# penn-graphics-research/claymore

Measured on AMD Instinct MI355X. Metric: particles*steps/sec, higher is better.
Workload: dtype f32

## Files before the change

claymore_amd/csrc/claymore_hip.hip:

```cpp
#include <hip/hip_runtime.h>

#include <algorithm>
#include <cmath>
#include <cstdio>
#include <cstdlib>
#include <chrono>
#include <cstring>
#include <string>
#include <vector>

#include "../../include/claymore_amd.h"
#include "mpm_kernels.hpp"
#include "mpm_readout.hpp"

using namespace mpm;

namespace {
constexpr int kHaloWords	 = 128;
constexpr int kStatusBlock = ST_WORDS + kHaloWords + kMaxVelSlots * kMaxVelStride;

struct Partition {
	int* table = nullptr;
	int* keys  = nullptr;
	int* count = nullptr;
// ... 26 lines not shown

}

struct SubstepEvents {
	hipEvent_t start = nullptr, g2p2g_start = nullptr, g2p2g_end = nullptr, end = nullptr;
};

struct mpm_ctx {
	mpm_config cfg {};
	GridCfg g {};
	int device = 0;
	hipStream_t s_compute = nullptr, s_comm = nullptr;
	SubstepEvents ev;
	hipEvent_t ev_comm = nullptr, ev_halo = nullptr;
	hipEvent_t ev_tag0 = nullptr, ev_tag1 = nullptr;
	bool lean_events = false;
	hipEvent_t ev_pending = nullptr;
	hipEvent_t ev_status = nullptr;
	bool grid_preupdated = false;
	bool grid_momentum = false;
	float preupdate_dt	 = 0.f;
	float fuse_dt_once	 = 0.f;
	bool rebuild_cleared = false;
	std::vector<hipEvent_t> ev_ring;
	Partition part[2];
	float* grid[2] = {nullptr, nullptr};
	int rollid	   = 0;
	int pbc = 0, nbc = 0, ebc = 0;
	int pbc_prev = 0;
	std::vector<Model> models;
	int* d_status		  = nullptr;
	int* h_status		  = nullptr;
	unsigned* d_maxvel	  = nullptr;
	float* h_maxvel		  = nullptr;
	double* d_totals	  = nullptr;
	unsigned long long* d_counter = nullptr;
	bool ready = false;
	int capacity_events = 0;
	long long books_bias = 0;
	bool has_collision = false;
	CollisionObject collision {};
	bool collision_running = false;
	float4* d_sdf = nullptr;
	mpm_timers timers {};
	float last_g2p2g_ms = 0.f;
	int* d_overlap	   = nullptr;
// ... 45 lines not shown
#define MPM_PAIR_DEFAULT 0xF
#endif
static int pair_mask() {
	static const int mask = [] {
		const char* e = std::getenv("MPM_G2P2G_PAIRS");
		return (e && *e ? (int) std::strtol(e, nullptr, 0) : MPM_PAIR_DEFAULT) & 0xF;
	}();
	return mask;
}

template<int M>
static auto g2p2g_for(bool pair) {
	return pair ? g2p2g_pair_kernel<M> : g2p2g_kernel<M>;
}

static int launch_prepare(mpm_ctx* ctx, int cur, int prev, bool list_is_out, int binoff_sel, const int* pbc_ptr, int nblocks_est, bool sort, bool publish);

static int fail(mpm_ctx* ctx, int code, const std::string& msg) {
	ctx->err = msg;
	return code;
}

static inline void phase_call(mpm_ctx* ctx) {
	if(ctx) ctx->group_summed = false;
}

template<typename T>
static hipError_t dalloc(T** p, size_t n) {
	return hipMalloc((void**) p, sizeof(T) * (n ? n : 1));
}

template<typename T>
struct DevScratch {
	T* p = nullptr;
	DevScratch() = default;
	DevScratch(const DevScratch&) = delete;
	DevScratch& operator=(const DevScratch&) = delete;
	~DevScratch() {
		if(p) hipFree(p);
	}
	hipError_t alloc(size_t n) { return dalloc(&p, n); }
};

template<typename T>
static hipError_t regrow(T** p, size_t old_n, size_t new_n, hipStream_t s) {
	T* q		 = nullptr;
	hipError_t e = hipMalloc((void**) &q, sizeof(T) * new_n);
// ... 79 lines not shown
	mc.cohesion			 = p.cohesion;
	mc.beta				 = p.beta;
	mc.yield_surface	 = p.yield_surface;
	mc.xi				 = p.xi;
	mc.msqr				 = p.msqr;
	mc.log_jp0			 = p.log_jp0;
	mc.volume_correction = p.volume_correction;
	mc.hardening_on		 = p.hardening_on;
	return mc;
}

int mpm_create(const mpm_config* cfg, int device, mpm_ctx** out) {
	if(!cfg || !out) return MPM_ERR_INVALID;
	if(cfg->domain_bits < 4 || cfg->domain_bits > 10) return MPM_ERR_INVALID;
	if(cfg->max_ppc < 1 || cfg->max_ppc > 128 || (cfg->max_ppc & (cfg->max_ppc - 1))) return MPM_ERR_INVALID;
	int ndev = 0;
	if(hipGetDeviceCount(&ndev) != hipSuccess || ndev == 0 || device < 0 || device >= ndev) {
		fprintf(stderr, "claymore_hip: no usable HIP device %d (found %d) - there is no CPU fallback\n", device, ndev);
		return MPM_ERR_DEVICE;
	}
	mpm_ctx* ctx = new mpm_ctx();
	ctx->cfg	 = *cfg;
	ctx->device	 = device;
	GridCfg& g	 = ctx->g;
	g.gbits		 = cfg->domain_bits - 2;
	g.G			 = 1 << g.gbits;
	g.ppb		 = cfg->max_ppc * 64;
	g.pid_bits	 = 0;
	while((1 << g.pid_bits) < g.ppb) g.pid_bits++;
	g.boundary = cfg->boundary_blocks;
	g.dx_inv   = (float) (1 << cfg->domain_bits);
	g.dx	   = 1.f / g.dx_inv;
	g.d_inv	   = 4.f * g.dx_inv * g.dx_inv;
	g.gravity  = cfg->gravity;
	g.cap	   = 0;
	int prio_lo = 0, prio_hi = 0;
	if(hipSetDevice(device) == hipSuccess) hipDeviceGetStreamPriorityRange(&prio_lo, &prio_hi);
	if(hipSetDevice(device) != hipSuccess || hipStreamCreateWithFlags(&ctx->s_compute, hipStreamNonBlocking) != hipSuccess || hipStreamCreateWithPriority(&ctx->s_comm, hipStreamNonBlocking, prio_hi) != hipSuccess) {
		delete ctx;
		return MPM_ERR_DEVICE;
	}
	if(hipEventCreate(&ctx->ev.start) != hipSuccess || hipEventCreate(&ctx->ev.end) != hipSuccess || hipEventCreate(&ctx->ev.g2p2g_start) != hipSuccess || hipEventCreate(&ctx->ev.g2p2g_end) != hipSuccess
	   || hipEventCreateWithFlags(&ctx->ev_comm, hipEventDisableTiming) != hipSuccess || hipEventCreateWithFlags(&ctx->ev_halo, hipEventDisableTiming) != hipSuccess
	   || hipEventCreateWithFlags(&ctx->ev_status, hipEventDisableTiming) != hipSuccess) {
		mpm_destroy(ctx);
		return MPM_ERR_DEVICE;
// ... 321 lines not shown
	const int* cur_keys	  = ctx->part[r].keys;
	const GridCfg& g = ctx->g;
	StepConst sk;
	sk.dtp	= dt * g.dx_inv;
	sk.dts	= dt * (4.f * g.dx_inv);
	sk.pred = next_dt * g.dx_inv;
	sk.am	= m.mc.mass * g.dx * g.dx * g.d_inv;
	const float cs = -next_dt * g.d_inv * g.dx;
	sk.ss	= StressScale {2.f * m.mc.mu * m.mc.volume * cs, m.mc.lambda * m.mc.volume * cs, m.mc.volume * cs};
	sk.refl_lim = sk.dts > 0.f ? (1.f / 3.f) / sk.dts : 3.0e38f;
	sk.jdiv		= g.dx * dt * g.d_inv;
	sk.jvisc	= g.dx * g.d_inv * m.mc.viscosity;
	const int nwg = nblocks_ptr ? hint_blocks(ctx, nblocks) : nblocks;
	auto kernel = g2p2g_for<3>(m.pair);
	switch(m.material) {
		case MPM_J_FLUID: kernel = g2p2g_for<0>(m.pair); break;
		case MPM_FIXED_COROTATED: kernel = g2p2g_for<1>(m.pair); break;
		case MPM_SAND: kernel = g2p2g_for<2>(m.pair); break;
		default: break;
	}
	kernel<<<nwg, kG2P2GThreads, 0, s>>>(ctx->g, v, cur_keys, ctx->grid[0], ctx->grid[1], block_list, only_flag, nblocks_ptr, nblocks, dt, next_dt, sk, ctx->d_status);
}

static int launch_clear(mpm_ctx* ctx, int flags) {
	if((flags & kClearRebuild) && !(flags & kClearP2G)) {
		if(ctx->rebuild_cleared) flags &= ~(kClearRebuild | kClearMaxVel);
		ctx->rebuild_cleared = false;
	}
	if(!(flags & (kClearP2G | kClearRebuild))) return MPM_OK;
	ClearArgs a {};
	a.flags	  = flags;
	a.nmodels = (int) ctx->models.size();
	for(int mi = 0; mi < a.nmodels; ++mi) a.out_count[mi] = ctx->models[mi].out_count, a.keep[mi] = ctx->models[mi].keep;
	a.p2g_grid	   = ctx->grid[1];
	a.status	   = ctx->d_status;
	a.max_vel_bits = ctx->d_maxvel;
	Partition& Pn  = ctx->part[ctx->rollid ^ 1];
	a.old_table	   = Pn.table;
	a.old_keys	   = Pn.keys;
	a.old_count	   = Pn.count;
	substep_clear_kernel<<<1024, 256, 0, ctx->s_compute>>>(ctx->g, a);
	return MPM_OK;
}
static int launch_g2p2g_prologue(mpm_ctx* ctx, bool with_rebuild = false, bool fused_update = false) {
	int rc = launch_clear(ctx, with_rebuild ? (kClearP2G | kClearRebuild | (fused_update ? kClearMaxVel : 0)) : kClearP2G);
	if(rc == MPM_OK && with_rebuild) ctx->rebuild_cleared = true;
	return rc;
}

static int launch_g2p2g(mpm_ctx* ctx, float dt, float next_dt, hipEvent_t e0, hipEvent_t e1, bool with_rebuild_clear = false, bool fused_update = false) {
	hipStream_t s = ctx->s_compute;
	int rc		  = launch_g2p2g_prologue(ctx, with_rebuild_clear, fused_update);
	if(rc) return rc;
	HIP_TRY(hipEventRecord(e0, s));
	if(ctx->pbc)
		for(auto& m: ctx->models) launch_g2p2g_model(ctx, m, nullptr, &ctx->d_status[ST_PBC], ctx->pbc, dt, next_dt, s);
	HIP_TRY(hipEventRecord(e1, s));
	return MPM_OK;
}

int mpm_g2p2g(mpm_ctx* ctx, float dt, float next_dt) {
	phase_call(ctx);
	if(!ctx || !ctx->ready) return MPM_ERR_NOT_READY;
	HIP_TRY(hipSetDevice(ctx->device));
	int rc = launch_g2p2g(ctx, dt, next_dt, ctx->ev.g2p2g_start, ctx->ev.g2p2g_end);
	if(rc) return rc;
	HIP_TRY(hipGetLastError());
	HIP_TRY(hipStreamSynchronize(ctx->s_compute));
	HIP_TRY(hipEventElapsedTime(&ctx->last_g2p2g_ms, ctx->ev.g2p2g_start, ctx->ev.g2p2g_end));
	ctx->timers.g2p2g_ms = ctx->last_g2p2g_ms;
	return MPM_OK;
}

static int launch_prepare(mpm_ctx* ctx, int cur, int prev, bool list_is_out, int binoff_sel, const int* pbc_ptr, int nblocks_est, bool sort, bool publish) {
	if(nblocks_est <= 0 && !publish) return MPM_OK;
	PrepareModels pm {};
	pm.n = (int) ctx->models.size();
	for(int mi = 0; mi < pm.n; ++mi) {
		Model& m		  = ctx->models[mi];
		pm.list[mi]		  = m.list[list_is_out ? (m.list_in ^ 1) : m.list_in];
// ... 74 lines not shown
		}
		for(auto& m: ctx->models) {
			for(int i = 0; i < 2; ++i) {
				HIP_TRY(regrow(&m.binoff[i], cap + 1, ncap + 1, s));
				HIP_TRY(regrow(&m.list[i], cap * (size_t) ctx->g.ppb, ncap * (size_t) ctx->g.ppb, s));
			}
			HIP_TRY(regrow(&m.size, cap + 1, ncap + 1, s));
			HIP_TRY(regrow(&m.row_of, cap + 1, ncap + 1, s));
			HIP_TRY(regrow(&m.out_count, cap + 1, ncap + 1, s));
			HIP_TRY(regrow(&m.keep, cap + 1, ncap + 1, s));
			HIP_TRY(regrow(&m.blockinfo, cap * (size_t) kInfoRow, ncap * (size_t) kInfoRow, s));
			if(m.pair)
				for(int i = 0; i < 2; ++i) HIP_TRY(regrow(&m.pairinfo[i], (cap + 1) * (size_t) kPairChunks, (ncap + 1) * (size_t) kPairChunks, s));
		}
		if(ctx->d_overlap) {
			HIP_TRY(regrow(&ctx->d_overlap, cap + 1, ncap + 1, s));
			HIP_TRY(regrow(&ctx->d_halo_list, cap + 1, ncap + 1, s));
			HIP_TRY(regrow(&ctx->d_inner_list, cap + 1, ncap + 1, s));
		}
		for(int p = 0; p < 32; ++p)
			if(ctx->d_send_ids[p]) HIP_TRY(regrow(&ctx->d_send_ids[p], cap + 1, ncap + 1, s));
		ctx->g.cap = (int) ncap;
		ctx->capacity_events++;
	}
	for(auto& m: ctx->models) {
		const size_t need = m.n / kBin + (size_t) ctx->g.cap + 1;
		if((size_t) m.bincount * 4 > m.bin_cap * 3 || need > m.bin_cap) {
			const size_t nb = std::max(need, (size_t) m.bincount * 4 > m.bin_cap * 3 ? m.bin_cap * 3 / 2 + 1 : m.bin_cap);
			HIP_TRY(hipDeviceSynchronize());
			for(int i = 0; i < 2; ++i) HIP_TRY(regrow(&m.bins[i], m.bin_cap * m.nch * kBin, nb * m.nch * kBin, s));
			m.bin_cap = nb;
			ctx->capacity_events++;
		}
	}
	return MPM_OK;
}

static void roll_partition(mpm_ctx* ctx) {
	for(auto& m: ctx->models) m.list_in ^= 1;
	ctx->rollid ^= 1;
}

static int check_books(mpm_ctx* ctx) {
	const long long gone = (long long) ctx->h_status[ST_LOST] + (long long) ctx->h_status[ST_DROPPED] + ctx->books_bias;
	long long added = 0, held = 0;
	for(size_t mi = 0; mi < ctx->models.size(); ++mi) {
		const Model& m = ctx->models[mi];
		added += (long long) m.n;
		held += (long long) m.bucketed;
		if(gone == 0 && (long long) m.bucketed != (long long) m.n)
			return fail(ctx, MPM_ERR_INTERNAL,
						"particle books of model " + std::to_string(mi) + " do not balance: " + std::to_string(m.bucketed) + " bucketed of " + std::to_string(m.n) +
							" added, none counted as lost or dropped");
	}
	if(held + gone != added)
// ... 65 lines not shown
	const float mv = std::sqrt(mv2);
	const float nd = mpm_compute_dt(ctx, mv, step_time, frame_time, dt_default);
	if(max_vel) *max_vel = mv;
	if(next_dt) *next_dt = nd;
	rc = launch_g2p2g(ctx, dt, nd, ctx->ev.g2p2g_start, ctx->ev.g2p2g_end, true);
	if(rc) return rc;
	hipStream_t s = ctx->s_compute;
	HIP_TRY(hipEventRecord(ctx->ev.start, s));
	rc = launch_rebuild(ctx);
	if(rc) return rc;
	HIP_TRY(hipEventRecord(ctx->ev.end, s));
	HIP_TRY(hipGetLastError());
	rc = finish_rebuild(ctx, nullptr);
	if(rc) return rc;
	HIP_TRY(hipEventElapsedTime(&ctx->last_g2p2g_ms, ctx->ev.g2p2g_start, ctx->ev.g2p2g_end));
	HIP_TRY(hipEventElapsedTime(&ctx->timers.partition_ms, ctx->ev.start, ctx->ev.end));
	ctx->timers.g2p2g_ms = ctx->last_g2p2g_ms;
	ctx->timers.total_ms = ctx->timers.grid_update_ms + ctx->timers.g2p2g_ms + ctx->timers.partition_ms;
	guard.armed = false;
	return MPM_OK;
}

int mpm_run_fixed(mpm_ctx* ctx, int nsteps, float dt) {
	phase_call(ctx);
	if(!ctx || !ctx->ready) return MPM_ERR_NOT_READY;
	HIP_TRY(hipSetDevice(ctx->device));
	hipStream_t s = ctx->s_compute;
	const int K = ctx->cfg.sync_interval > 0 ? std::min(ctx->cfg.sync_interval, 64) : 8;
	FlagGuard guard {ctx};
	while((int) ctx->ev_ring.size() < 3 * K + 1) {
		hipEvent_t e = nullptr;
		HIP_TRY(hipEventCreate(&e));
		ctx->ev_ring.push_back(e);
	}
	{
		int rc = grow_capacity(ctx);
		if(rc) return rc;
	}
	double acc_grid = 0, acc_g2p2g = 0, acc_part = 0, acc_total = 0;
	int in_window = 0;
	for(int it = 0; it < nsteps; ++it) {
		hipEvent_t* ev = &ctx->ev_ring[3 * in_window];
		if(in_window == 0) HIP_TRY(hipEventRecord(ev[0], s));
		int rc = launch_grid_update(ctx, dt);
		if(rc) return rc;
		const bool fuse_next = it + 1 < nsteps;
		rc = launch_g2p2g(ctx, dt, dt, ev[1], ev[2], true, fuse_next);
		if(rc) return rc;
		rc = launch_rebuild(ctx, fuse_next ? dt : 0.f);
		if(rc) return rc;
		HIP_TRY(hipEventRecord(ev[3], s));
		roll_partition(ctx);
		++in_window;
		const bool tight = ctx->cfg.grow && (long long) ctx->ebc * 10 > (long long) ctx->g.cap * 7 &&
						   (size_t) ctx->g.cap < (size_t) ctx->g.G * ctx->g.G * ctx->g.G;
		if(in_window == K || it + 1 == nsteps || tight) {
			HIP_TRY(hipGetLastError());
			rc = sync_counts(ctx, nullptr);
			if(rc) return rc;
			if(std::isinf(host_maxvel(ctx))) return fail(ctx, MPM_ERR_NONFINITE, "Maximum velocity is infinity");
			for(int w = 0; w < in_window; ++w) {
				hipEvent_t* e = &ctx->ev_ring[3 * w];
				float t_grid = 0, t_g = 0, t_part = 0, t_tot = 0;
				HIP_TRY(hipEventElapsedTime(&t_grid, e[0], e[1]));
				HIP_TRY(hipEventElapsedTime(&t_g, e[1], e[2]));
				HIP_TRY(hipEventElapsedTime(&t_part, e[2], e[3]));
				HIP_TRY(hipEventElapsedTime(&t_tot, e[0], e[3]));
				acc_grid += t_grid;
				acc_g2p2g += t_g;
				acc_part += t_part;
				acc_total += t_tot;
				ctx->last_g2p2g_ms = t_g;
			}
			in_window = 0;
		}
	}
	if(nsteps > 0) {
		ctx->timers.grid_update_ms = (float) (acc_grid / nsteps);
		ctx->timers.g2p2g_ms	   = (float) (acc_g2p2g / nsteps);
		ctx->timers.partition_ms   = (float) (acc_part / nsteps);
		ctx->timers.total_ms	   = (float) (acc_total / nsteps);
	}
	guard.armed = false;
	return MPM_OK;
}

int mpm_state_kind(void) {
	return MPM_STATE_B;
}

const char* mpm_build_info(void) {
	return "claymore_hip abi7 state=b"
#ifdef MPM_EXPERIMENT
		   " experiment=MPM_EXPERIMENT"
#ifdef MPM_HACK_STALE_INTERIOR
		   ",MPM_HACK_STALE_INTERIOR"
#endif
#ifdef MPM_G2P2G_STATS
		   ",MPM_G2P2G_STATS"
#endif
#else
		   " experiment=none"
#endif
		;
}

int mpm_last_g2p2g_ms(mpm_ctx* ctx, float* ms) {
	if(!ctx || !ms) return MPM_ERR_INVALID;
	*ms = ctx->last_g2p2g_ms;
	return MPM_OK;
}

int mpm_get_counts(mpm_ctx* ctx, mpm_counts* counts) {
	if(!ctx || !ctx->ready || !counts) return MPM_ERR_NOT_READY;
	memset(counts, 0, sizeof(*counts));
// ... 68 lines not shown
	if(!ctx) return MPM_ERR_INVALID;
	if(!ctx->has_collision) return fail(ctx, MPM_ERR_INVALID, "no collision object installed");
	if(time) *time = ctx->collision.time;
	if(running) *running = ctx->collision_running ? 1 : 0;
	return MPM_OK;
}

int mpm_get_capacity(mpm_ctx* ctx, int64_t* block_capacity, int64_t* bin_capacity, int* growth_events) {
	if(!ctx || !ctx->ready) return MPM_ERR_NOT_READY;
	if(block_capacity) *block_capacity = ctx->g.cap;
	if(bin_capacity)
		for(size_t i = 0; i < ctx->models.size() && i < 8; ++i) bin_capacity[i] = (int64_t) ctx->models[i].bin_cap;
	if(growth_events) *growth_events = ctx->capacity_events;
	return MPM_OK;
}

int mpm_get_diagnostics(mpm_ctx* ctx, mpm_diagnostics* d) {
	if(!ctx || !ctx->ready || !d) return MPM_ERR_NOT_READY;
	memset(d, 0, sizeof(*d));
	d->lost_particles = ctx->h_status[ST_LOST];
	d->discarded_p2g  = ctx->h_status[ST_ARENA];
	d->overflow_flags = ctx->h_status[ST_OVERFLOW];
	d->dropped_particles = ctx->h_status[ST_DROPPED];
#ifdef MPM_G2P2G_STATS
	for(int i = 0; i < 4; ++i) d->reserved[i] = ctx->h_status[24 + i];
#endif
	return MPM_OK;
}

int mpm_get_timers(mpm_ctx* ctx, mpm_timers* t) {
	if(!ctx || !t) return MPM_ERR_INVALID;
	*t = ctx->timers;
	return MPM_OK;
}

static int readout_particles(mpm_ctx* ctx, int model, ReadoutKind kind, float* const host[3], size_t* n) {
	HIP_TRY(hipSetDevice(ctx->device));
	hipStream_t s	 = ctx->s_compute;
	Model& m		 = ctx->models[model];
	const size_t cap = std::min(*n, m.n);
	DevScratch<float> scratch[3];
	ReadoutOut out {{m.d_xyz, nullptr, nullptr}, cap, ctx->d_counter, 0.0, nullptr};
	for(int c = 1; c < 3; ++c)
		if(host[c]) {
			HIP_TRY(scratch[c].alloc(kReadoutWidth[kind][c] * cap));
			out.col[c] = scratch[c].p;
// ... 166 lines not shown
```

claymore_amd/csrc/mpm_checkpoint.inc:

```

namespace {
struct CkptModel {
	int32_t material, nch, list_in, layout;
	int64_t n, bincount, bincount_src, bucketed;
};
struct CkptHeader {
	uint64_t magic;
	int32_t domain_bits, max_ppc, nmodels, rollid;
	int32_t pbc, nbc, ebc, prev_count;
	uint64_t total_bytes;
	uint64_t param_hash;
	int32_t prev_pbc;
	int32_t grid_velocity;
	CkptModel models[8];
};
constexpr uint64_t kCkptMagic = 0x3754504b434d504dull;

struct CkptLayout {
	size_t cur_keys, prev_keys, grid, end;
	size_t size[8], row_of[8], binoff_src[8], binoff_dst[8], bins[8], lists[8], pairinfo[8];
};
static CkptLayout ckpt_layout(const CkptHeader& h) {
	CkptLayout L {};
	size_t o	= sizeof(CkptHeader);
// ... 304 lines not shown
			if(e == hipSuccess) e = hipMemcpyAsync(d_packed, in + L.lists[mi], sizeof(int) * (size_t) M.bucketed, hipMemcpyHostToDevice, s);
			int* d_info = nullptr;
			if(e == hipSuccess && M.pair) e = dalloc(&d_info, (size_t) h.pbc * kPairChunks);
			if(e == hipSuccess && M.pair) e = hipMemcpyAsync(d_info, in + L.pairinfo[mi], sizeof(int) * (size_t) h.pbc * kPairChunks, hipMemcpyHostToDevice, s);
			if(e == hipSuccess) {
				unpack_lists_kernel<<<h.pbc, 64, 0, s>>>(ctx->g.ppb, M.size, M.row_of, d_off, M.list[M.list_in], d_packed, M.pair ? 1 : 0, M.pairinfo[0], d_info);
				e = hipGetLastError();
			}
			if(e == hipSuccess) e = hipStreamSynchronize(s);
			hipFree(d_off);
			hipFree(d_packed);
			hipFree(d_info);
			if(e != hipSuccess) return fail(ctx, MPM_ERR_DEVICE, std::string("checkpoint: ") + hipGetErrorString(e));
		}
	}
	{
		HIP_TRY(hipMemcpyAsync(ctx->h_status, ctx->d_status, sizeof(int) * ST_WORDS, hipMemcpyDeviceToHost, s));
		HIP_TRY(hipStreamSynchronize(s));
		int* st		= ctx->h_status;
		st[ST_PBC] = h.pbc, st[ST_NBC] = h.nbc, st[ST_EBC] = h.ebc, st[ST_PBCPREV] = h.prev_pbc;
		ctx->pbc_prev = h.prev_pbc;
		st[ST_CNT_P] = st[ST_CNT_N] = st[ST_CNT_E] = 0;
		st[ST_OVERFLOW] = st[ST_NONFINITE] = 0;
		for(int mi = 0; mi < kMaxModels; ++mi) {
			st[ST_BINS0 + mi]	 = mi < h.nmodels ? (int) h.models[mi].bincount : 0;
			st[ST_BINSPREV + mi] = mi < h.nmodels ? (int) h.models[mi].bincount_src : 0;
			st[ST_PART0 + mi]	 = mi < h.nmodels ? (int) h.models[mi].bucketed : 0;
		}
		{
			long long added = 0, held = 0;
			for(int mi = 0; mi < h.nmodels; ++mi) added += (long long) h.models[mi].n, held += (long long) h.models[mi].bucketed;
			ctx->books_bias = added - held - ((long long) st[ST_LOST] + (long long) st[ST_DROPPED]);
		}
		HIP_TRY(hipMemcpyAsync(ctx->d_status, st, sizeof(int) * ST_WORDS, hipMemcpyHostToDevice, s));
		HIP_TRY(hipMemsetAsync(ctx->d_maxvel, 0, sizeof(unsigned) * kMaxVelSlots * kMaxVelStride, s));
	}
	{
		int rc = launch_prepare(ctx, r, n, false, r, &ctx->d_status[ST_PBC], h.pbc, false, false);
		if(rc) return rc;
	}
	HIP_TRY(hipGetLastError());
	HIP_TRY(hipStreamSynchronize(s));
	ctx->halo_tagged = false;
	return MPM_OK;
}
```

claymore_amd/csrc/mpm_group.inc:

```
#include <rccl/rccl.h>
#include <dlfcn.h>

#include <atomic>
#include <condition_variable>
#include <mutex>

namespace {

struct Rccl {
	void* lib = nullptr;
	ncclResult_t (*GetUniqueId)(ncclUniqueId*)																  = nullptr;
	ncclResult_t (*CommInitRank)(ncclComm_t*, int, ncclUniqueId, int)											  = nullptr;
	ncclResult_t (*CommDestroy)(ncclComm_t)																	  = nullptr;
	ncclResult_t (*CommAbort)(ncclComm_t)																		  = nullptr;
	ncclResult_t (*CommCount)(const ncclComm_t, int*)															  = nullptr;
	ncclResult_t (*AllGather)(const void*, void*, size_t, ncclDataType_t, ncclComm_t, hipStream_t)				  = nullptr;
	ncclResult_t (*AllReduce)(const void*, void*, size_t, ncclDataType_t, ncclRedOp_t, ncclComm_t, hipStream_t) = nullptr;
	ncclResult_t (*Send)(const void*, size_t, ncclDataType_t, int, ncclComm_t, hipStream_t)					  = nullptr;
	ncclResult_t (*Recv)(void*, size_t, ncclDataType_t, int, ncclComm_t, hipStream_t)							  = nullptr;
	ncclResult_t (*GroupStart)()																				  = nullptr;
	ncclResult_t (*GroupEnd)()																					  = nullptr;
	const char* (*GetErrorString)(ncclResult_t)																  = nullptr;
};
Rccl* rccl() {
// ... 537 lines not shown
	hipFree(g->d_scalar);
	if(g->ev_sent) hipEventDestroy(g->ev_sent);
	if(g->ev_done) hipEventDestroy(g->ev_done);
	if(g->ev_keys) hipEventDestroy(g->ev_keys);
	if(g->ev_kdone) hipEventDestroy(g->ev_kdone);
	for(const SubstepEvents& ev: g->ev2)
		for(hipEvent_t e: {ev.start, ev.g2p2g_start, ev.g2p2g_end, ev.end})
			if(e) hipEventDestroy(e);
	delete g;
}

const char* mpm_group_transport(const mpm_group* g) {
	if(!g) return "";
	if(!g->hub) return "rccl";
	return g->hub->peer_direct ? "peer-direct" : "device-copy";
}
const char* mpm_group_last_error(const mpm_group* g) {
	return g ? g->err.c_str() : "null group";
}

int mpm_group_initial_setup(mpm_group* g) {
	if(!g || !g->ctx) return MPM_ERR_INVALID;
	g->ctx->group_summed = false;
	GRP_TRY(mpm_initial_setup(g->ctx));
	int rc = grp_tag(g);
	if(rc) return rc;
	rc = grp_exchange_halo(g, 0, false, 0.f, 0.f, g->ctx->ev);
	if(rc) return rc;
	GRP_TRY(mpm_sync(g->ctx));
	g->ctx->group_summed = true;
	return MPM_OK;
}

int mpm_group_resume(mpm_group* g) {
	if(!g || !g->ctx) return MPM_ERR_INVALID;
	g->ctx->group_summed = false;
	if(g->aborted) return gfail(g, MPM_ERR_DEVICE, "the RCCL communicator was aborted after an error");
	mpm_ctx* ctx = g->ctx;
	if(!ctx->ready) return gfail(g, MPM_ERR_NOT_READY, "mpm_group_resume: the context holds no state (initial set-up or mpm_checkpoint_load first)");
	ctx->group_summed = false;
	GRP_TRY(mpm_sync(ctx));
	ctx->halo_tagged = false;
	g->pad			 = 0;
	int rc			 = grp_tag(g);
	if(rc) return rc;
	GRP_TRY(mpm_sync(ctx));
	ctx->group_summed = true;
	return MPM_OK;
}

namespace {
int grp_substep_begin(mpm_group* g, float dt, float next_dt, bool device_sized, const SubstepEvents& ev) {
	GRP_TRY(mgsp_begin(g->ctx, dt, next_dt, device_sized, ev));
	return MPM_OK;
}
int grp_substep_tail(mpm_group* g, const SubstepEvents& ev) {
	mpm_ctx* ctx  = g->ctx;
	const int pad = g->pad;
	int rc		  = grp_key_buffers(g);
	if(rc) return rc;
	if(g->overlap_tag) {
		for(hipEvent_t* e: {&ctx->ev_tag0, &ctx->ev_tag1})
			if(!*e) GRP_HIP(hipEventCreateWithFlags(e, hipEventDisableTiming));
// ... 20 lines not shown
int grp_substep_enqueue(mpm_group* g, float dt, float next_dt, const SubstepEvents& ev) {
	int rc = grp_exchange_halo(g, 1, true, dt, next_dt, ev);
	return rc ? rc : grp_substep_tail(g, ev);
}
int grp_substep_wait(mpm_group* g, const SubstepEvents& ev, float* max_vel_sqr, bool* truncated) {
	mpm_ctx* ctx = g->ctx;
	int mx		 = 0;
	float mv	 = 0.f;
	GRP_TRY(mgsp_end_wait(ctx, g->rank, g->send_counts, &g->n_halo_blocks, &mx, &mv, ev));
	g->send_counts[g->rank] = 0;
	if(max_vel_sqr) *max_vel_sqr = mv;
	g->g2p2g_ms_sum += ctx->last_g2p2g_ms;
	g->steps++;
	const int pad = g->pad_enqueued;
	*truncated	  = mx > pad;
	if(*truncated || grp_pad_close(g, mx, pad)) g->pad = std::max(g->pad, grp_pad_for(g, mx));
	return MPM_OK;
}
}

int mpm_group_substep(mpm_group* g, float dt, float next_dt, float* max_vel_sqr) {
	if(!g || !g->ctx) return MPM_ERR_INVALID;
	g->ctx->group_summed = false;
	const SubstepEvents& ev = g->ctx->ev;
	int rc					= grp_substep_begin(g, dt, next_dt, false, ev);
	if(rc) return rc;
	rc = grp_substep_enqueue(g, dt, next_dt, ev);
	if(rc) return rc;
	bool truncated = false;
	rc			   = grp_substep_wait(g, ev, max_vel_sqr, &truncated);
	if(rc) return rc;
	if(truncated) {
		g->retags++;
		if((rc = grp_tag(g))) return rc;
	}
	g->ctx->group_summed = true;
	return MPM_OK;
}

int mpm_group_run_fixed(mpm_group* g, int nsteps, float dt) {
	if(!g || !g->ctx) return MPM_ERR_INVALID;
	mpm_ctx* ctx	  = g->ctx;
	ctx->group_summed = false;
	bool pending = false;
	bool retagged = false;
	bool lean_prev_end = false;
	auto bail = [&](int rc) {
		ctx->fuse_dt_once = 0.f, ctx->grid_preupdated = false, ctx->rebuild_cleared = false;
		if(pending) hipEventSynchronize(ctx->ev_pending ? ctx->ev_pending : ctx->ev_status);
		ctx->lean_events = false;
		return rc;
	};
	auto finish = [&](int par, bool may_retag) {
		SubstepEvents ev = g->ev2[par];
		if(ctx->lean_events) ev.start = lean_prev_end ? g->ev2[par ^ 1].end : ev.g2p2g_start;
		lean_prev_end  = ctx->lean_events;
		float mv	   = 0.f;
		bool truncated = false;
		int rc		   = grp_substep_wait(g, ev, &mv, &truncated);
		pending		   = false;
		if(rc == MPM_OK && (std::isinf(mv) || std::isnan(mv))) rc = gfail(g, MPM_ERR_NONFINITE, "Maximum velocity is infinity");
		if(rc == MPM_OK && truncated) {
			if(!may_retag) GRP_HIP(hipStreamSynchronize(ctx->s_compute));
			rc = grp_tag(g);
			g->retags++;
			retagged = true;
// ... 25 lines not shown
}

float mpm_group_compute_dt(const mpm_group* g, float max_vel, float cur, float next, float dt_default) {
	if(!g || !g->ctx) return 0.f;
	if(next < cur) return 0.f;
	float dt = dt_default;
	if(max_vel > 0.f) {
		max_vel = g->ctx->g.dx * 0.3f / max_vel;
		if(max_vel < dt_default) dt = max_vel;
	}
	if(cur + dt >= next) {
		dt = next - cur;
	} else {
		max_vel = (next - cur) * 0.51f;
		if(max_vel < dt) dt = max_vel;
	}
	return dt;
}

int mpm_group_main_loop(mpm_group* g, int frames, int fps, float dt_default, void (*on_frame)(int frame, void* user), void* user, int* steps_out) {
	if(!g || !g->ctx || frames < 0 || fps < 1) return MPM_ERR_INVALID;
	mpm_ctx* ctx			= g->ctx;
	ctx->group_summed		= false;
	const float seconds_pf	= 1.f / (float) fps;
	float next_dt			= mpm_group_compute_dt(g, 0.f, 0.f, seconds_pf, dt_default);
	int steps				= 0;
	for(int frame = 1; frame <= frames; ++frame) {
		const float next_time = seconds_pf;
		float cur_time		  = 0.f;
		while(cur_time < next_time) {
			const float dt = next_dt;
			if(!(dt > 0.f)) return gfail(g, MPM_ERR_INVALID, "time step is not positive");
			float mv2 = 0.f;
			GRP_TRY(mpm_grid_update(ctx, dt, &mv2));
			int rc = grp_all_reduce_max(g, &mv2);
			if(rc) return rc;
			if(std::isinf(mv2) || std::isnan(mv2)) return gfail(g, MPM_ERR_NONFINITE, "Maximum velocity is infinity");
			next_dt = mpm_group_compute_dt(g, std::sqrt(mv2), cur_time + dt, next_time, dt_default);
			if(!(next_dt > 0.f)) next_dt = mpm_group_compute_dt(g, std::sqrt(mv2), 0.f, seconds_pf, dt_default);
			GRP_TRY(mpm_g2p2g_halo(ctx, dt, next_dt));
			rc = grp_exchange_halo(g, 1, true, dt, next_dt, ctx->ev);
			if(rc) return rc;
			GRP_TRY(mpm_rebuild_partition(ctx, nullptr));
			rc = grp_tag(g);
			if(rc) return rc;
			g->g2p2g_ms_sum += ctx->last_g2p2g_ms;
// ... 83 lines not shown
```

claymore_amd/csrc/mpm_kernels.hpp:

```cpp
#pragma once
#include <hip/hip_runtime.h>
#include <type_traits>

#include "mpm_device_math.hpp"
#include "mpm_collision.hpp"

namespace mpm {

constexpr int kBin		  = 64;
constexpr int kG2P2GThreads = 64;
constexpr int kMaxModels  = 8;
constexpr int kSortKeys		= 216;
constexpr int kKeyBits		= 8;
constexpr int kStay		  = 13;

enum {
	ST_PBC = 0, ST_NBC = 1, ST_EBC = 2, ST_OVERFLOW = 3, ST_LOST = 4, ST_ARENA = 5, ST_DROPPED = 6, ST_NONFINITE = 7, ST_BINS0 = 8, ST_PART0 = 16,
	 ST_CNT_P = 29, ST_CNT_N = 30, ST_CNT_E = 31, ST_BINSPREV = 32, ST_PBCPREV = 40, ST_WORDS = 64
};

struct GridCfg {
	int G;
	int gbits;
	int ppb;
	int pid_bits;
	int boundary;
	int cap;
	float dx, dx_inv, d_inv, gravity;
};

__device__ __forceinline__ bool key_ok(const GridCfg& c, int x, int y, int z) {
	return ((unsigned) x < (unsigned) c.G) & ((unsigned) y < (unsigned) c.G) & ((unsigned) z < (unsigned) c.G);
}
__device__ __forceinline__ size_t key_index(const GridCfg& c, int x, int y, int z) {
	return ((size_t) x << (2 * c.gbits)) | ((size_t) y << c.gbits) | (size_t) z;
}
__device__ __forceinline__ int table_query(const GridCfg& c, const int* __restrict__ table, int x, int y, int z) {
	return key_ok(c, x, y, z) ? table[key_index(c, x, y, z)] : -1;
}
__device__ __forceinline__ void table_insert(const GridCfg& c, int* table, int* keys, int* count, int x, int y, int z, int* status) {
	if(!key_ok(c, x, y, z)) return;
// ... 267 lines not shown
	int n;
	int* list[kMaxModels];
	const int* size[kMaxModels];
	const int* row_of[kMaxModels];
	const int* binoff_src[kMaxModels];
	int* blockinfo[kMaxModels];
	const int* keep[kMaxModels];
	int* pairinfo[kMaxModels];
	const int* pairhand[kMaxModels];
};
template<bool SORT>
__global__ __launch_bounds__(64) void prepare_blocks_kernel(GridCfg cfg, PrepareModels pm, const int* __restrict__ pbc_ptr, const int* __restrict__ cur_table, const int* __restrict__ cur_keys, const int* __restrict__ prev_table, int* __restrict__ publish, int* __restrict__ part_count) {
	constexpr int kPrepChunk = kListChunk;
	__shared__ int s_sorted[kPairChunkMax];
	__shared__ int s_cnt[256];
	__shared__ int s_cur[256];
	const int lane = threadIdx.x;
	if(publish && blockIdx.x == 0 && lane == 0) {
		const int ebc	 = publish[ST_CNT_P] + publish[ST_CNT_N] + publish[ST_CNT_E];
		publish[ST_EBC] = ebc;
		*part_count		 = ebc;
	}
	const int pbc = min(*pbc_ptr, cfg.cap);
	for(int b = blockIdx.x; b < pbc; b += gridDim.x) {
	const int kx = cur_keys[3 * b], ky = cur_keys[3 * b + 1], kz = cur_keys[3 * b + 2];
	int size0 = 0, row0 = 0, keep0 = -2, hand0 = 0;
	if constexpr(SORT) {
		if(pm.n > 0) {
			size0 = pm.size[0][b];
			row0  = pm.row_of[0][b];
			if(pm.keep[0]) keep0 = pm.keep[0][row0];
			if(pm.pairinfo[0]) hand0 = pm.pairhand[0][(size_t) row0 * kPairChunks + (lane & (kPairChunks - 1))];
		}
	}
	int srcno = -1, other = -1;
	if(lane < 27) {
		int ox, oy, oz;
		dir_components(lane, ox, oy, oz);
		srcno = table_query(cfg, prev_table, kx + ox, ky + oy, kz + oz);
	} else if(lane < 54) {
		int ox, oy, oz;
		dir_components(lane - 27, ox, oy, oz);
		other = table_query(cfg, cur_table, kx - ox, ky - oy, kz - oz);
	} else if(lane < 62) {
		const int lb = lane - 54;
		other		 = table_query(cfg, cur_table, kx + ((lb >> 2) & 1), ky + ((lb >> 1) & 1), kz + (lb & 1));
	}
	const int key_shift		= cfg.pid_bits;
	const int tag_shift		= cfg.pid_bits + kKeyBits;
	const unsigned rec_mask = (1u << (tag_shift + 5)) - 1u;
	for(int m = 0; m < pm.n; ++m) {
		int info = other;
		if constexpr(SORT) {
		const int size = __builtin_amdgcn_readfirstlane(m == 0 ? size0 : pm.size[m][b]);
		const int row  = __builtin_amdgcn_readfirstlane(m == 0 ? row0 : pm.row_of[m][b]);
		int* list	   = pm.list[m] + (size_t) row * cfg.ppb;
		const int tail	= size & (kPrepChunk - 1);
		int* pairinfo	= pm.pairinfo[m] ? pm.pairinfo[m] + (size_t) b * kPairChunks : nullptr;
		const int kept	= m == 0 ? keep0 : (pm.keep[m] ? pm.keep[m][row] : -2);
// ... 159 lines not shown
			if(big) {
#pragma unroll
				for(int it = 0; it < kPairTailMerge / 64; ++it)
					if(it * 64 + lane < n1g) list[chunk0 + kPrepChunk + it * 64 + lane] = s_sorted[kPrepChunk + it * 64 + lane];
			}
			if(lane == 0) pairinfo[chunk0 / kPrepChunk] = pf;
			__syncthreads();
		};
		if(pairinfo && same && lane < kPairChunks) pairinfo[lane] = m == 0 ? hand0 : pm.pairhand[m][(size_t) row * kPairChunks + lane];
		for(int chunk0 = 0; chunk0 < size && !same; chunk0 += kPrepChunk) {
			const int left = size - chunk0;
			const int nrec = (pairinfo && left > kPrepChunk && left <= kPairChunkMax) ? left : min(kPrepChunk, left);
			if(chunk0) load_chunk(chunk0, min(kPrepChunk, nrec));
			if(pairinfo)
				sort_chunk_pairs(chunk0, nrec);
			else
				sort_chunk(chunk0, nrec);
			if(nrec > kPrepChunk) break;
		}
		}
		if constexpr(!SORT) {
			if(lane < 27) info = srcno >= 0 ? pm.binoff_src[m][srcno] : -1;
		}
		pm.blockinfo[m][(size_t) b * kInfoRow + lane] = info;
	}
	}
}

}
#include "mpm_g2p2g.hpp"
#include "mpm_g2p2g_pair.hpp"
namespace mpm {

struct RebuildModels {
	int n;
	const int* out_count[kMaxModels];
	int* size[kMaxModels];
	int* row_of[kMaxModels];
	int* binoff[kMaxModels];
	long long bin_cap[kMaxModels];
};

enum { kClearP2G = 1, kClearRebuild = 2, kClearMaxVel = 4 };
struct ClearArgs {
	int flags;
	int nmodels;
	int* out_count[kMaxModels];
	int* keep[kMaxModels];
	float* p2g_grid;
	int* status;
	unsigned* max_vel_bits;
	int* old_table;
	const int* old_keys;
	const int* old_count;
};
__global__ __launch_bounds__(256) void substep_clear_kernel(GridCfg cfg, ClearArgs a) {
	const int tid = blockIdx.x * 256 + threadIdx.x, nthreads = gridDim.x * 256;
	if(a.flags & kClearP2G) {
		const int nbc = min(a.status[ST_NBC], cfg.cap), ebc = min(a.status[ST_EBC], cfg.cap);
		float4* g	  = reinterpret_cast<float4*>(a.p2g_grid);
		for(int i = tid; i < nbc * 64; i += nthreads) g[i] = make_float4(0.f, 0.f, 0.f, 0.f);
		for(int m = 0; m < a.nmodels; ++m)
			for(int i = tid; i <= ebc; i += nthreads) a.out_count[m][i] = 0, a.keep[m][i] = -1;
	}
	if(a.flags & kClearRebuild) {
		const int n = min(*a.old_count, cfg.cap);
		for(int i = tid; i < n; i += nthreads) a.old_table[key_index(cfg, a.old_keys[3 * i], a.old_keys[3 * i + 1], a.old_keys[3 * i + 2])] = -1;
		if(blockIdx.x == gridDim.x - 1) {
			if(threadIdx.x < kMaxModels) {
				a.status[ST_BINSPREV + threadIdx.x] = a.status[ST_BINS0 + threadIdx.x];
				a.status[ST_BINS0 + threadIdx.x]	= 0;
				a.status[ST_PART0 + threadIdx.x]	= 0;
			}
			if(threadIdx.x >= 8 && threadIdx.x < 11) a.status[ST_CNT_P + threadIdx.x - 8] = 0;
			if(threadIdx.x == 11) a.status[ST_PBCPREV] = a.status[ST_PBC];
			if(threadIdx.x >= 64 && threadIdx.x < 64 + kMaxVelSlots) {
				unsigned* slot = a.max_vel_bits + (threadIdx.x - 64) * kMaxVelStride;
				if(*slot >= 0x7f800000u) a.status[ST_NONFINITE] = 1;
				if(a.flags & kClearMaxVel) *slot = 0u;
			}
		}
	}
}

__global__ __launch_bounds__(1024) void compact_blocks_kernel(GridCfg cfg, RebuildModels rm, const int* __restrict__ old_keys, int* __restrict__ new_keys, int* __restrict__ new_table, int* __restrict__ status) {
	__shared__ int s_part[kMaxModels];
	const int ebc = min(status[ST_EBC], cfg.cap);
	for(int b0 = blockIdx.x * blockDim.x; b0 < ebc; b0 += gridDim.x * blockDim.x) {
		const int b = b0 + threadIdx.x;
		int c[kMaxModels];
		bool any = false;
		for(int m = 0; m < rm.n; ++m) {
			c[m] = b < ebc ? rm.out_count[m][b] : 0;
			if(c[m] > cfg.ppb) {
				atomicAdd(&status[ST_DROPPED], c[m] - cfg.ppb);
				c[m] = cfg.ppb;
			}
			any |= c[m] > 0;
		}
		__syncthreads();
		if(threadIdx.x < kMaxModels) s_part[threadIdx.x] = 0;
		__syncthreads();
		for(int m = 0; m < rm.n; ++m) {
			int t = c[m];
#pragma unroll
			for(int off = 32; off > 0; off >>= 1) t += __shfl_xor(t, off);
			if((threadIdx.x & 63) == 0 && t) atomicAdd(&s_part[m], t);
		}
		__syncthreads();
		if((int) threadIdx.x < rm.n && s_part[threadIdx.x]) atomicAdd(&status[ST_PART0 + threadIdx.x], s_part[threadIdx.x]);
		const int nb = block_append(&status[ST_CNT_P], any ? 1 : 0);
		int kx = 0, ky = 0, kz = 0;
		if(any) {
			kx = old_keys[3 * b], ky = old_keys[3 * b + 1], kz = old_keys[3 * b + 2];
			new_keys[3 * nb]					  = kx;
			new_keys[3 * nb + 1]				  = ky;
			new_keys[3 * nb + 2]				  = kz;
			new_table[key_index(cfg, kx, ky, kz)] = nb;
		}
		for(int m = 0; m < rm.n; ++m) {
			const int nbins = any ? (c[m] + kBin - 1) / kBin : 0;
			const int first = block_append(&status[ST_BINS0 + m], nbins);
			if(any) {
				const bool fits = (long long) first + nbins <= rm.bin_cap[m];
				if(!fits) atomicOr(&status[ST_OVERFLOW], 4);
				rm.size[m][nb]	 = fits ? c[m] : 0;
				rm.row_of[m][nb] = b;
				rm.binoff[m][nb] = (nbins && fits) ? first : 0;
			}
		}
	}
}

template<int LO, int HI>
__global__ __launch_bounds__(256) void register_blocks_kernel(GridCfg cfg, const int* __restrict__ pbc_ptr, const int* __restrict__ base2_ptr, int* counter, int* publish, int* table, int* keys, int* status) {
	constexpr int W	   = HI - LO + 1;
	constexpr int NOFF = W * W * W;
	constexpr int LPB  = NOFF <= 8 ? 8 : 32;
	const int pbc	   = min(*pbc_ptr, cfg.cap);
	const int base	   = *pbc_ptr + (base2_ptr ? *base2_ptr : 0);
	if(publish && blockIdx.x == 0 && threadIdx.x == 0) *publish = base;
	const long long total = (long long) pbc * LPB;
	const long long bound = (total + blockDim.x - 1) / blockDim.x * blockDim.x;
	for(long long t = (long long) blockIdx.x * blockDim.x + threadIdx.x; t < bound; t += (long long) gridDim.x * blockDim.x) {
		const int b = (int) (t / LPB), o = (int) (t % LPB);
		bool claim	= false;
		int x = 0, y = 0, z = 0;
		size_t i = 0;
		if(t < total && o < NOFF) {
			x = keys[3 * b] + LO + o / (W * W);
			y = keys[3 * b + 1] + LO + (o / W) % W;
			z = keys[3 * b + 2] + LO + o % W;
			if(key_ok(cfg, x, y, z)) {
				i = key_index(cfg, x, y, z);
				if(table[i] == -1) claim = atomicCAS(&table[i], -1, -2) == -1;
			}
		}
		const int idx = base + block_append(counter, claim ? 1 : 0);
		if(claim) {
			if(idx < cfg.cap) {
				table[i]		  = idx;
				keys[3 * idx]	  = x;
				keys[3 * idx + 1] = y;
				keys[3 * idx + 2] = z;
			} else {
				table[i] = -1;
				atomicOr(&status[ST_OVERFLOW], 1);
			}
		}
	}
}

template<bool UPDATE, bool COLLIDE = false>
__global__ __launch_bounds__(256) void carry_grid_kernel(GridCfg cfg, const int* __restrict__ status, const int* __restrict__ new_keys, const int* __restrict__ old_table, const float* __restrict__ p2g_grid, float* __restrict__ grid, float dt, unsigned* __restrict__ max_vel_bits, std::conditional_t<COLLIDE, CollisionArgs, NoCollision> col) {
	static_assert(UPDATE || !COLLIDE, "the collision object belongs to the grid update");
	const int nbc	  = min(status[ST_CNT_P] + status[ST_CNT_N], cfg.cap);
	const int old_nbc = min(status[ST_NBC], cfg.cap);
	const int lane = threadIdx.x & 63;
	float vel_sqr  = 0.f;
	for(int nb = blockIdx.x * 4 + (threadIdx.x >> 6); nb < nbc; nb += gridDim.x * 4) {
		const int kx = new_keys[3 * nb], ky = new_keys[3 * nb + 1], kz = new_keys[3 * nb + 2];
		const int old = table_query(cfg, old_table, kx, ky, kz);
		float4 v	  = {0.f, 0.f, 0.f, 0.f};
		if(old >= 0 && old < old_nbc) {
			const float* s = p2g_grid + (size_t) old * 256;
			v			   = {s[lane], s[64 + lane], s[128 + lane], s[192 + lane]};
		}
		if constexpr(COLLIDE) {
			if(v.x > 0.0f) vel_sqr = fmaxf(vel_sqr, grid_cell_collision(cfg, col, kx, ky, kz, lane, dt, v));
		} else if constexpr(UPDATE) {
			if(v.x > 0.0f) {
				const bool wx = kx < cfg.boundary || kx >= cfg.G - cfg.boundary;
				const bool wy = ky < cfg.boundary || ky >= cfg.G - cfg.boundary;
				const bool wz = kz < cfg.boundary || kz >= cfg.G - cfg.boundary;
				const float mass_inv = 1.f / v.x;
				const float v0		 = wx ? 0.0f : v.y * mass_inv;
				const float v1		 = (wy ? 0.0f : v.z * mass_inv) + cfg.gravity * dt;
				const float v2		 = wz ? 0.0f : v.w * mass_inv;
				v.y					 = v0;
				v.z					 = v1;
				v.w					 = v2;
				float q				 = v0 * v0 + v1 * v1 + v2 * v2;
				if(q != q) q = __builtin_inff();
				vel_sqr = fmaxf(vel_sqr, q);
			}
// ... 182 lines not shown
```

Baseline: 34.00 billion.

## Reuse previous block partition when the active block set is unchanged

Adds a device-side check (partition_same_kernel) that detects whether the set of occupied blocks and the overflow counters match the previous step. When they match, compaction keeps block order, block registration is skipped, carry_grid uses identity indices instead of hash lookups, and the neighbor-info build reuses the previously stored rows instead of querying tables. The goal is to remove rebuild overhead in steady-state steps. The cost is an extra kernel and more status words. Correctness now depends on the sameness check covering every way the layout can change.

After: 34.36 billion (median of 2 runs). Within noise of the previous version (+1.1%).

```diff
diff --git a/claymore_amd/csrc/claymore_hip.hip b/claymore_amd/csrc/claymore_hip.hip
--- a/claymore_amd/csrc/claymore_hip.hip
+++ b/claymore_amd/csrc/claymore_hip.hip
@@ -72,6 +72,8 @@
 	float preupdate_dt	 = 0.f;
 	float fuse_dt_once	 = 0.f;
 	bool rebuild_cleared = false;
+	bool reuse_enabled = true;
+	bool reuse_armed   = false;
 	std::vector<hipEvent_t> ev_ring;
 	Partition part[2];
 	float* grid[2] = {nullptr, nullptr};
@@ -163,7 +165,7 @@
 }
 
 static inline void phase_call(mpm_ctx* ctx) {
-	if(ctx) ctx->group_summed = false;
+	if(ctx) ctx->group_summed = false, ctx->reuse_armed = false;
 }
 
 template<typename T>
@@ -289,6 +291,10 @@
 	mpm_ctx* ctx = new mpm_ctx();
 	ctx->cfg	 = *cfg;
 	ctx->device	 = device;
+	{
+		const char* e	   = std::getenv("MPM_PARTITION_REUSE");
+		ctx->reuse_enabled = !(e && *e) || std::strtol(e, nullptr, 0) != 0;
+	}
 	GridCfg& g	 = ctx->g;
 	g.gbits		 = cfg->domain_bits - 2;
 	g.G			 = 1 << g.gbits;
@@ -656,7 +662,7 @@
 	kernel<<<nwg, kG2P2GThreads, 0, s>>>(ctx->g, v, cur_keys, ctx->grid[0], ctx->grid[1], block_list, only_flag, nblocks_ptr, nblocks, dt, next_dt, sk, ctx->d_status);
 }
 
-static int launch_clear(mpm_ctx* ctx, int flags) {
+static int launch_clear(mpm_ctx* ctx, int flags, bool reuse = false) {
 	if((flags & kClearRebuild) && !(flags & kClearP2G)) {
 		if(ctx->rebuild_cleared) flags &= ~(kClearRebuild | kClearMaxVel);
 		ctx->rebuild_cleared = false;
@@ -673,23 +679,31 @@
 	a.old_table	   = Pn.table;
 	a.old_keys	   = Pn.keys;
 	a.old_count	   = Pn.count;
+	a.reuse		   = reuse ? 1 : 0;
 	substep_clear_kernel<<<1024, 256, 0, ctx->s_compute>>>(ctx->g, a);
 	return MPM_OK;
 }
-static int launch_g2p2g_prologue(mpm_ctx* ctx, bool with_rebuild = false, bool fused_update = false) {
-	int rc = launch_clear(ctx, with_rebuild ? (kClearP2G | kClearRebuild | (fused_update ? kClearMaxVel : 0)) : kClearP2G);
+static int launch_g2p2g_prologue(mpm_ctx* ctx, bool with_rebuild = false, bool fused_update = false, bool reuse = false) {
+	int rc = launch_clear(ctx, with_rebuild ? (kClearP2G | kClearRebuild | (fused_update ? kClearMaxVel : 0)) : kClearP2G, with_rebuild && reuse);
 	if(rc == MPM_OK && with_rebuild) ctx->rebuild_cleared = true;
 	return rc;
 }
 
-static int launch_g2p2g(mpm_ctx* ctx, float dt, float next_dt, hipEvent_t e0, hipEvent_t e1, bool with_rebuild_clear = false, bool fused_update = false) {
+static int launch_g2p2g(mpm_ctx* ctx, float dt, float next_dt, hipEvent_t e0, hipEvent_t e1, bool with_rebuild_clear = false, bool fused_update = false, bool reuse = false) {
 	hipStream_t s = ctx->s_compute;
-	int rc		  = launch_g2p2g_prologue(ctx, with_rebuild_clear, fused_update);
+	int rc		  = launch_g2p2g_prologue(ctx, with_rebuild_clear, fused_update, reuse);
 	if(rc) return rc;
 	HIP_TRY(hipEventRecord(e0, s));
 	if(ctx->pbc)
 		for(auto& m: ctx->models) launch_g2p2g_model(ctx, m, nullptr, &ctx->d_status[ST_PBC], ctx->pbc, dt, next_dt, s);
 	HIP_TRY(hipEventRecord(e1, s));
+	if(with_rebuild_clear && reuse) {
+		SameModels sm {};
+		sm.n = (int) ctx->models.size();
+		for(int mi = 0; mi < sm.n; ++mi) sm.out_count[mi] = ctx->models[mi].out_count;
+		const int ebc_est = std::min(ctx->g.cap, ctx->ebc + ctx->ebc / 16 + 1024);
+		partition_same_kernel<<<std::max(1u, cdiv(ebc_est, 1024)), 1024, 0, s>>>(ctx->g, sm, ctx->d_status);
+	}
 	return MPM_OK;
 }
 
@@ -810,6 +824,7 @@
 			if(ctx->d_send_ids[p]) HIP_TRY(regrow(&ctx->d_send_ids[p], cap + 1, ncap + 1, s));
 		ctx->g.cap = (int) ncap;
 		ctx->capacity_events++;
+		ctx->reuse_armed = false;
 	}
 	for(auto& m: ctx->models) {
 		const size_t need = m.n / kBin + (size_t) ctx->g.cap + 1;
@@ -819,6 +834,7 @@
 			for(int i = 0; i < 2; ++i) HIP_TRY(regrow(&m.bins[i], m.bin_cap * m.nch * kBin, nb * m.nch * kBin, s));
 			m.bin_cap = nb;
 			ctx->capacity_events++;
+			ctx->reuse_armed = false;
 		}
 	}
 	return MPM_OK;
@@ -930,8 +946,10 @@
 }
 
 int mpm_run_fixed(mpm_ctx* ctx, int nsteps, float dt) {
+	const bool was_armed = ctx && ctx->reuse_armed;
 	phase_call(ctx);
 	if(!ctx || !ctx->ready) return MPM_ERR_NOT_READY;
+	ctx->reuse_armed = was_armed;
 	HIP_TRY(hipSetDevice(ctx->device));
 	hipStream_t s = ctx->s_compute;
 	const int K = ctx->cfg.sync_interval > 0 ? std::min(ctx->cfg.sync_interval, 64) : 8;
@@ -953,15 +971,18 @@
 		int rc = launch_grid_update(ctx, dt);
 		if(rc) return rc;
 		const bool fuse_next = it + 1 < nsteps;
-		rc = launch_g2p2g(ctx, dt, dt, ev[1], ev[2], true, fuse_next);
+		const bool near_cap = ctx->cfg.grow && (long long) ctx->ebc * 10 > (long long) ctx->g.cap * 7 &&
+							  (size_t) ctx->g.cap < (size_t) ctx->g.G * ctx->g.G * ctx->g.G;
+		const bool reuse	= ctx->reuse_enabled && ctx->reuse_armed && !near_cap;
+		rc = launch_g2p2g(ctx, dt, dt, ev[1], ev[2], true, fuse_next, reuse);
 		if(rc) return rc;
 		rc = launch_rebuild(ctx, fuse_next ? dt : 0.f);
 		if(rc) return rc;
 		HIP_TRY(hipEventRecord(ev[3], s));
 		roll_partition(ctx);
+		ctx->reuse_armed = true;
 		++in_window;
-		const bool tight = ctx->cfg.grow && (long long) ctx->ebc * 10 > (long long) ctx->g.cap * 7 &&
-						   (size_t) ctx->g.cap < (size_t) ctx->g.G * ctx->g.G * ctx->g.G;
+		const bool tight = near_cap;
 		if(in_window == K || it + 1 == nsteps || tight) {
 			HIP_TRY(hipGetLastError());
 			rc = sync_counts(ctx, nullptr);
@@ -998,7 +1019,7 @@
 }
 
 const char* mpm_build_info(void) {
-	return "claymore_hip abi7 state=b"
+	return "claymore_hip abi7 state=b switches=MPM_G2P2G_PAIRS,MPM_PARTITION_REUSE"
 #ifdef MPM_EXPERIMENT
 		   " experiment=MPM_EXPERIMENT"
 #ifdef MPM_HACK_STALE_INTERIOR
@@ -1113,6 +1134,8 @@
 	d->discarded_p2g  = ctx->h_status[ST_ARENA];
 	d->overflow_flags = ctx->h_status[ST_OVERFLOW];
 	d->dropped_particles = ctx->h_status[ST_DROPPED];
+	d->reserved[0]		 = ctx->h_status[ST_SAME_HITS];
+	d->reserved[1]		 = ctx->h_status[ST_SAME];
 #ifdef MPM_G2P2G_STATS
 	for(int i = 0; i < 4; ++i) d->reserved[i] = ctx->h_status[24 + i];
 #endif
diff --git a/claymore_amd/csrc/mpm_checkpoint.inc b/claymore_amd/csrc/mpm_checkpoint.inc
--- a/claymore_amd/csrc/mpm_checkpoint.inc
+++ b/claymore_amd/csrc/mpm_checkpoint.inc
@@ -350,6 +350,7 @@
 		ctx->pbc_prev = h.prev_pbc;
 		st[ST_CNT_P] = st[ST_CNT_N] = st[ST_CNT_E] = 0;
 		st[ST_OVERFLOW] = st[ST_NONFINITE] = 0;
+		st[ST_SAME] = 0;
 		for(int mi = 0; mi < kMaxModels; ++mi) {
 			st[ST_BINS0 + mi]	 = mi < h.nmodels ? (int) h.models[mi].bincount : 0;
 			st[ST_BINSPREV + mi] = mi < h.nmodels ? (int) h.models[mi].bincount_src : 0;
diff --git a/claymore_amd/csrc/mpm_group.inc b/claymore_amd/csrc/mpm_group.inc
--- a/claymore_amd/csrc/mpm_group.inc
+++ b/claymore_amd/csrc/mpm_group.inc
@@ -583,6 +583,7 @@
 int mpm_group_initial_setup(mpm_group* g) {
 	if(!g || !g->ctx) return MPM_ERR_INVALID;
 	g->ctx->group_summed = false;
+	g->ctx->reuse_armed = false;
 	GRP_TRY(mpm_initial_setup(g->ctx));
 	int rc = grp_tag(g);
 	if(rc) return rc;
@@ -596,10 +597,12 @@
 int mpm_group_resume(mpm_group* g) {
 	if(!g || !g->ctx) return MPM_ERR_INVALID;
 	g->ctx->group_summed = false;
+	g->ctx->reuse_armed = false;
 	if(g->aborted) return gfail(g, MPM_ERR_DEVICE, "the RCCL communicator was aborted after an error");
 	mpm_ctx* ctx = g->ctx;
 	if(!ctx->ready) return gfail(g, MPM_ERR_NOT_READY, "mpm_group_resume: the context holds no state (initial set-up or mpm_checkpoint_load first)");
 	ctx->group_summed = false;
+	ctx->reuse_armed = false;
 	GRP_TRY(mpm_sync(ctx));
 	ctx->halo_tagged = false;
 	g->pad			 = 0;
@@ -666,6 +669,7 @@
 int mpm_group_substep(mpm_group* g, float dt, float next_dt, float* max_vel_sqr) {
 	if(!g || !g->ctx) return MPM_ERR_INVALID;
 	g->ctx->group_summed = false;
+	g->ctx->reuse_armed = false;
 	const SubstepEvents& ev = g->ctx->ev;
 	int rc					= grp_substep_begin(g, dt, next_dt, false, ev);
 	if(rc) return rc;
@@ -686,6 +690,7 @@
 	if(!g || !g->ctx) return MPM_ERR_INVALID;
 	mpm_ctx* ctx	  = g->ctx;
 	ctx->group_summed = false;
+	ctx->reuse_armed = false;
 	bool pending = false;
 	bool retagged = false;
 	bool lean_prev_end = false;
@@ -757,6 +762,7 @@
 	if(!g || !g->ctx || frames < 0 || fps < 1) return MPM_ERR_INVALID;
 	mpm_ctx* ctx			= g->ctx;
 	ctx->group_summed		= false;
+	ctx->reuse_armed = false;
 	const float seconds_pf	= 1.f / (float) fps;
 	float next_dt			= mpm_group_compute_dt(g, 0.f, 0.f, seconds_pf, dt_default);
 	int steps				= 0;
diff --git a/claymore_amd/csrc/mpm_kernels.hpp b/claymore_amd/csrc/mpm_kernels.hpp
--- a/claymore_amd/csrc/mpm_kernels.hpp
+++ b/claymore_amd/csrc/mpm_kernels.hpp
@@ -16,7 +16,8 @@
 
 enum {
 	ST_PBC = 0, ST_NBC = 1, ST_EBC = 2, ST_OVERFLOW = 3, ST_LOST = 4, ST_ARENA = 5, ST_DROPPED = 6, ST_NONFINITE = 7, ST_BINS0 = 8, ST_PART0 = 16,
-	 ST_CNT_P = 29, ST_CNT_N = 30, ST_CNT_E = 31, ST_BINSPREV = 32, ST_PBCPREV = 40, ST_WORDS = 64
+	 ST_CNT_P = 29, ST_CNT_N = 30, ST_CNT_E = 31, ST_BINSPREV = 32, ST_PBCPREV = 40,
+	ST_SAME = 48, ST_SAME_HITS = 49, ST_SAME_SNAP = 50, ST_WORDS = 64
 };
 
 struct GridCfg {
@@ -330,8 +331,11 @@
 		*part_count		 = ebc;
 	}
 	const int pbc = min(*pbc_ptr, cfg.cap);
+	const bool reuse = SORT && publish && pm.n > 0 && __builtin_amdgcn_readfirstlane(publish[ST_SAME]) != 0;
+	if(reuse && blockIdx.x == 0 && lane == 0) publish[ST_SAME_HITS] += 1;
 	for(int b = blockIdx.x; b < pbc; b += gridDim.x) {
-	const int kx = cur_keys[3 * b], ky = cur_keys[3 * b + 1], kz = cur_keys[3 * b + 2];
+	int kx = 0, ky = 0, kz = 0;
+	if(!reuse) kx = cur_keys[3 * b], ky = cur_keys[3 * b + 1], kz = cur_keys[3 * b + 2];
 	int size0 = 0, row0 = 0, keep0 = -2, hand0 = 0;
 	if constexpr(SORT) {
 		if(pm.n > 0) {
@@ -342,7 +346,13 @@
 		}
 	}
 	int srcno = -1, other = -1;
-	if(lane < 27) {
+	if(reuse) {
+		const int* row = pm.blockinfo[0] + (size_t) b * kInfoRow;
+		if(lane < 27)
+			srcno = row[53 - lane];
+		else if(lane < 62)
+			other = row[lane];
+	} else if(lane < 27) {
 		int ox, oy, oz;
 		dir_components(lane, ox, oy, oz);
 		srcno = table_query(cfg, prev_table, kx + ox, ky + oy, kz + oz);
@@ -548,7 +558,7 @@
 		if constexpr(!SORT) {
 			if(lane < 27) info = srcno >= 0 ? pm.binoff_src[m][srcno] : -1;
 		}
-		pm.blockinfo[m][(size_t) b * kInfoRow + lane] = info;
+		if(!reuse || lane < 27) pm.blockinfo[m][(size_t) b * kInfoRow + lane] = info;
 	}
 	}
 }
@@ -579,6 +589,7 @@
 	int* old_table;
 	const int* old_keys;
 	const int* old_count;
+	int reuse;
 };
 __global__ __launch_bounds__(256) void substep_clear_kernel(GridCfg cfg, ClearArgs a) {
 	const int tid = blockIdx.x * 256 + threadIdx.x, nthreads = gridDim.x * 256;
@@ -600,6 +611,8 @@
 			}
 			if(threadIdx.x >= 8 && threadIdx.x < 11) a.status[ST_CNT_P + threadIdx.x - 8] = 0;
 			if(threadIdx.x == 11) a.status[ST_PBCPREV] = a.status[ST_PBC];
+			if(threadIdx.x == 12) a.status[ST_SAME] = a.reuse;
+			if(threadIdx.x >= 13 && threadIdx.x < 16) a.status[ST_SAME_SNAP + threadIdx.x - 13] = a.status[threadIdx.x == 13 ? ST_OVERFLOW : threadIdx.x == 14 ? ST_LOST : ST_ARENA];
 			if(threadIdx.x >= 64 && threadIdx.x < 64 + kMaxVelSlots) {
 				unsigned* slot = a.max_vel_bits + (threadIdx.x - 64) * kMaxVelStride;
 				if(*slot >= 0x7f800000u) a.status[ST_NONFINITE] = 1;
@@ -609,9 +622,32 @@
 	}
 }
 
+struct SameModels {
+	int n;
+	const int* out_count[kMaxModels];
+};
+__global__ __launch_bounds__(1024) void partition_same_kernel(GridCfg cfg, SameModels sm, int* __restrict__ status) {
+	__shared__ int s_offered;
+	if(threadIdx.x == 0) s_offered = status[ST_SAME];
+	__syncthreads();
+	if(s_offered == 0) return;
+	const int ebc = min(status[ST_EBC], cfg.cap), pbc = status[ST_PBC];
+	bool differs = false;
+	for(int b = blockIdx.x * blockDim.x + threadIdx.x; b < ebc; b += gridDim.x * blockDim.x) {
+		bool any = false;
+		for(int m = 0; m < sm.n; ++m) any |= sm.out_count[m][b] > 0;
+		differs |= any != (b < pbc);
+	}
+	if(blockIdx.x == 0 && threadIdx.x == 0)
+		differs |= status[ST_OVERFLOW] != status[ST_SAME_SNAP] || status[ST_LOST] != status[ST_SAME_SNAP + 1] || status[ST_ARENA] != status[ST_SAME_SNAP + 2] || status[ST_EBC] > cfg.cap;
+	if(__syncthreads_or(differs) && threadIdx.x == 0) status[ST_SAME] = 0;
+}
+
 __global__ __launch_bounds__(1024) void compact_blocks_kernel(GridCfg cfg, RebuildModels rm, const int* __restrict__ old_keys, int* __restrict__ new_keys, int* __restrict__ new_table, int* __restrict__ status) {
 	__shared__ int s_part[kMaxModels];
 	const int ebc = min(status[ST_EBC], cfg.cap);
+	const bool same = status[ST_SAME] != 0;
+	if(same && blockIdx.x == 0 && threadIdx.x < 3) status[ST_CNT_P + threadIdx.x] = threadIdx.x == 0 ? status[ST_PBC] : status[ST_PBC + threadIdx.x] - status[ST_PBC + threadIdx.x - 1];
 	for(int b0 = blockIdx.x * blockDim.x; b0 < ebc; b0 += gridDim.x * blockDim.x) {
 		const int b = b0 + threadIdx.x;
 		int c[kMaxModels];
@@ -635,9 +671,9 @@
 		}
 		__syncthreads();
 		if((int) threadIdx.x < rm.n && s_part[threadIdx.x]) atomicAdd(&status[ST_PART0 + threadIdx.x], s_part[threadIdx.x]);
-		const int nb = block_append(&status[ST_CNT_P], any ? 1 : 0);
+		const int nb = same ? b : block_append(&status[ST_CNT_P], any ? 1 : 0);
 		int kx = 0, ky = 0, kz = 0;
-		if(any) {
+		if(same ? b < ebc : any) {
 			kx = old_keys[3 * b], ky = old_keys[3 * b + 1], kz = old_keys[3 * b + 2];
 			new_keys[3 * nb]					  = kx;
 			new_keys[3 * nb + 1]				  = ky;
@@ -663,6 +699,7 @@
 	constexpr int W	   = HI - LO + 1;
 	constexpr int NOFF = W * W * W;
 	constexpr int LPB  = NOFF <= 8 ? 8 : 32;
+	if(status[ST_SAME]) return;
 	const int pbc	   = min(*pbc_ptr, cfg.cap);
 	const int base	   = *pbc_ptr + (base2_ptr ? *base2_ptr : 0);
 	if(publish && blockIdx.x == 0 && threadIdx.x == 0) *publish = base;
@@ -702,11 +739,12 @@
 	static_assert(UPDATE || !COLLIDE, "the collision object belongs to the grid update");
 	const int nbc	  = min(status[ST_CNT_P] + status[ST_CNT_N], cfg.cap);
 	const int old_nbc = min(status[ST_NBC], cfg.cap);
+	const bool same	  = status[ST_SAME] != 0;
 	const int lane = threadIdx.x & 63;
 	float vel_sqr  = 0.f;
 	for(int nb = blockIdx.x * 4 + (threadIdx.x >> 6); nb < nbc; nb += gridDim.x * 4) {
 		const int kx = new_keys[3 * nb], ky = new_keys[3 * nb + 1], kz = new_keys[3 * nb + 2];
-		const int old = table_query(cfg, old_table, kx, ky, kz);
+		const int old = same ? nb : table_query(cfg, old_table, kx, ky, kz);
 		float4 v	  = {0.f, 0.f, 0.f, 0.f};
 		if(old >= 0 && old < old_nbc) {
 			const float* s = p2g_grid + (size_t) old * 256;
```
